# sdoira/U96-SLAM

Hardware: AMD Instinct MI355X
Metric: Mpix-disparities/s (higher is better)
Workload: dtype u8

## Files before the change

### u96-slam_amd/csrc/sbm_api.hip

```cpp
#include <stdio.h>
#include <stdlib.h>
#include <string.h>

#include <algorithm>
#include <mutex>
#include <new>

#include "sbm_handle.h"

using namespace sbm;

enum BmStage { kBmPrefilter, kBmSad, kBmBorder, kBmLr, kBmSpeckle, kBmTotal, kBmStageCount };
enum BmMark { kBmBegin, kBmPrefiltered, kBmMatched, kBmChecked, kBmEnd, kBmMarkCount };
static const char* const kBmNames[] = {"prefilter", "sad", "border", "lrcheck", "speckle", "total"};
StageTable sbm::bm_stages() { return stage_table<kBmStageCount, 0>(kBmNames); }
static_assert(kBmMarkCount == sbm_handle::kMarks, "the ring holds one event per mark");

extern "C" {

void sbm_params_default(sbm_params* p, int num_disparities, int block_size) {
  if (!p) return;
  memset(p, 0, sizeof(*p));
  p->prefilter_type = SBM_PREFILTER_XSOBEL;
  p->prefilter_size = 9;
// ... 346 lines not shown
  if (n <= 0) return SBM_ERR_BATCH;
  const sbm_params& p = h->p;
  BmPlan pl;
  const int st = bm_plan_geom(p, n, width, height, &pl);
  if (st != SBM_OK) return st;
  DeviceScope dscope(h->device);
  HIPCHK(h, dscope.enter());
  bool inplace = false;
  if (pl.in_envelope) HIPCHK(h, mqsad_inplace_ok(h->stream, &inplace));
  bm_plan_launches(p, inplace, &pl);
  const Geom& g = pl.g;
  size_t ho_flags = 0;
  const size_t ho_bytes = sad_fast_handoff_bytes(pl, &ho_flags);
  const int st2 = ensure_scratch(h, n, width, height, g.pitch, g.want_cost, pl.speckle, ho_bytes, ho_flags);
  if (st2 != SBM_OK) return st2;
  h->last = g; h->have_last = true;
  h->bm.ho_links = 0;
  if (pl.any_rows) snprintf(h->last_kernel, sizeof(h->last_kernel), "%s", pl.kernel);

  const uint8_t* dl = (const uint8_t*)d_left;
  const uint8_t* dr = (const uint8_t*)d_right;
  uint8_t *pf_l = h->bm.pf_l.as<uint8_t>(), *pf_r = h->bm.pf_r.as<uint8_t>();
  int16_t* disp_pre = h->bm.disp_pre.as<int16_t>();
  int32_t* cost = h->bm.cost.as<int32_t>();
  int16_t* out = (int16_t*)d_disp;

  h->instr = h->profiling && h->ev_ok && (h->profiling != 3 || (h->ncall & 3u) == 0);
  mark(h, kBmBegin);
  if (pl.any_rows) {
    if (p.prefilter_type == SBM_PREFILTER_XSOBEL) {
      HIPCHK(h, launch_prefilter(dl, dr, pf_l, pf_r, g, h->stream));
    } else {
      HIPCHK(h, h->bm.vsum.grow((size_t)2 * h->bm.n * width * height * sizeof(uint16_t), h->stream));
      HIPCHK(h, launch_prefilter_norm(dl, dr, pf_l, pf_r, h->bm.vsum.as<uint16_t>(), g, p.prefilter_size, h->stream));
    }
  }
  mark(h, kBmPrefiltered);
  if (pl.sad == kSadFast) {
    HIPCHK(h, launch_sad_fast(pf_l, pf_r, disp_pre, cost, pl, ho_bytes ? h->bm.handoff.p : nullptr, ho_bytes ? ++h->bm.ho_epoch : 0u,
                              &h->bm.ho_links, h->stream));
    h->bm.ho_slots = (size_t)h->bm.ho_links;
    if (pl.wide_borders) {
      HIPCHK(h, launch_sad_wide(pf_l, pf_r, disp_pre, cost, g, pl.wide_l[0], pl.wide_l[1], h->stream));
      HIPCHK(h, launch_sad_wide(pf_l, pf_r, disp_pre, cost, g, pl.wide_r[0], pl.wide_r[1], h->stream));
    }
  } else if (pl.sad == kSadWide) {
    HIPCHK(h, launch_sad_wide(pf_l, pf_r, disp_pre, cost, g, 0, g.xend, h->stream));
  } else if (pl.sad == kSadGeneric) {
    HIPCHK(h, launch_sad_generic(pf_l, pf_r, disp_pre, cost, g, 0, g.xend, h->stream));
  }
  mark(h, kBmMatched);
  HIPCHK(h, launch_lrcheck(disp_pre, cost, out, h->bm.lr_keys.as<unsigned long long>(), g, p.disp12_max_diff, h->stream));
  mark(h, kBmChecked);
  if (pl.speckle) HIPCHK(h, launch_speckle(out, h->bm.spk, g, pl.spk, p.speckle_window_size, h->stream));
  mark(h, kBmEnd);
  if (h->instr) h->calls++;
  h->ncall++;
  if (sync || h->profiling == 1) HIPCHK(h, hipStreamSynchronize(h->stream));
  return SBM_OK;
}

int sbm_debug_plan(const sbm_params* p, int n, int width, int height, int inplace_ok, void* out, size_t out_bytes) {
  if (!p || !out) return SBM_ERR_NULL;
  if (out_bytes != sizeof(BmPlan)) return SBM_ERR_SIZE;
  if (n <= 0) return SBM_ERR_BATCH;
  BmPlan pl;
  const int st = bm_plan(*p, n, width, height, inplace_ok != 0, &pl);
  if (st == SBM_OK) memcpy(out, &pl, sizeof(pl));
  return st;
}

int sbm_debug_handoff_bytes(const sbm_params* p, int n, int width, int height, int inplace_ok, uint64_t* out) {
  if (!p || !out) return SBM_ERR_NULL;
  if (n <= 0) return SBM_ERR_BATCH;
  BmPlan pl;
  const int st = bm_plan(*p, n, width, height, inplace_ok != 0, &pl);
  if (st != SBM_OK) return st;
  size_t flags = 0;
  out[0] = sad_fast_handoff_bytes(pl, &flags);
  out[1] = flags;
  return SBM_OK;
}

int sbm_rect_map_device(sbm_handle* h, const sbm_rect_cam* cam, int width, int height, void* d_map, int sync) {
  if (!h || !cam || !d_map) return SBM_ERR_NULL;
  if (width <= 0 || height <= 0 || width > 32767 || height > 32767) return SBM_ERR_SIZE;
  DeviceScope dscope(h->device);
  HIPCHK(h, dscope.enter());
  HIPCHK(h, launch_rect_map(*cam, width, height, (int16_t*)d_map, h->stream));
  if (sync) HIPCHK(h, hipStreamSynchronize(h->stream));
  return SBM_OK;
}

int sbm_rect_remap_device(sbm_handle* h, int n, const void* d_src, const void* d_map, int width, int height, void* d_dst,
                          int sync) {
  if (!h || !d_src || !d_map || !d_dst) return SBM_ERR_NULL;
  if (n <= 0) return SBM_ERR_BATCH;
  if (width <= 0 || height <= 0 || width > 32767 || height > 32767) return SBM_ERR_SIZE;
  if (((size_t)width * height + 1023) / 1024 > 65535) return SBM_ERR_UNSUPPORTED;
  DeviceScope dscope(h->device);
  HIPCHK(h, dscope.enter());
  HIPCHK(h, launch_rect_remap((const uint8_t*)d_src, (const int16_t*)d_map, (uint8_t*)d_dst, n, width, height, h->stream));
  if (sync) HIPCHK(h, hipStreamSynchronize(h->stream));
  return SBM_OK;
}

int sbm_prefilter_device(sbm_handle* h, int n, const void* d_src, int width, int height, int flavour, int cap,
                         void* d_dst, int sync) {
  if (!h || !d_src || !d_dst) return SBM_ERR_NULL;
  if (n <= 0) return SBM_ERR_BATCH;
  if (width <= 0 || height <= 0) return SBM_ERR_SIZE;
  if (flavour != SBM_PREFILTER_FLAVOUR_CV && flavour != SBM_PREFILTER_FLAVOUR_RTL) return SBM_ERR_PREFILTER_TYPE;
  if (flavour == SBM_PREFILTER_FLAVOUR_CV && (cap < 1 || cap > 63)) return SBM_ERR_PREFILTER_CAP;
  if (n > 65534 || height > 65535 * 4) return SBM_ERR_UNSUPPORTED;
  DeviceScope dscope(h->device);
  HIPCHK(h, dscope.enter());
  HIPCHK(h, launch_prefilter_dense((const uint8_t*)d_src, (uint8_t*)d_dst, n, width, height,
                                   flavour == SBM_PREFILTER_FLAVOUR_RTL, cap, h->stream));
  if (sync) HIPCHK(h, hipStreamSynchronize(h->stream));
  return SBM_OK;
}

int sbm_disparity_to_float_device(sbm_handle* h, int n, const void* d_disp, int width, int height, void* d_out, int sync) {
  if (!h || !d_disp || !d_out) return SBM_ERR_NULL;
  if (n <= 0) return SBM_ERR_BATCH;
  if (width <= 0 || height <= 0) return SBM_ERR_SIZE;
  DeviceScope dscope(h->device);
  HIPCHK(h, dscope.enter());
  HIPCHK(h, launch_disp_to_float((const int16_t*)d_disp, (float*)d_out, (size_t)n * width * height, h->stream));
  if (sync) HIPCHK(h, hipStreamSynchronize(h->stream));
  return SBM_OK;
}

int sbm_decimate_device(sbm_handle* h, int n, const void* d_disp, int width, int height, int scale, void* d_out, int sync) {
  if (!h || !d_disp || !d_out) return SBM_ERR_NULL;
  if (n <= 0) return SBM_ERR_BATCH;
  if (width <= 0 || height <= 0 || scale <= 0) return SBM_ERR_SIZE;
  DeviceScope dscope(h->device);
  HIPCHK(h, dscope.enter());
  HIPCHK(h, launch_decimate((const int16_t*)d_disp, (int16_t*)d_out, n, width, height, scale, h->stream));
  if (sync) HIPCHK(h, hipStreamSynchronize(h->stream));
  return SBM_OK;
}

int sbm_reproject_device(sbm_handle* h, int n, const void* d_disp, int width, int height, int scale,
                         const sbm_stereo_model* model, int apply_local, void* d_xyz, int sync) {
  if (!h || !d_disp || !d_xyz || !model) return SBM_ERR_NULL;
  if (n <= 0) return SBM_ERR_BATCH;
  if (width <= 0 || height <= 0 || scale <= 0) return SBM_ERR_SIZE;
  DeviceScope dscope(h->device);
  HIPCHK(h, dscope.enter());
  HIPCHK(h, launch_reproject((const int16_t*)d_disp, (float*)d_xyz, n, width, height, scale, *model, apply_local, h->stream));
  if (sync) HIPCHK(h, hipStreamSynchronize(h->stream));
  return SBM_OK;
}

int sbm_keypoints3d_device(sbm_handle* h, const void* d_disp, int width, int height, const void* d_kpts, int nk,
                           const sbm_stereo_model* model, float min_depth, float max_depth, void* d_xyz, int sync) {
  if (!h || !d_disp || !model || (nk > 0 && (!d_kpts || !d_xyz))) return SBM_ERR_NULL;
  if (width <= 0 || height <= 0 || nk < 0) return SBM_ERR_SIZE;
  DeviceScope dscope(h->device);
  HIPCHK(h, dscope.enter());
  HIPCHK(h, launch_keypoints3d((const int16_t*)d_disp, (const float*)d_kpts, (float*)d_xyz, width, height, nk, *model,
                               min_depth, max_depth, h->stream));
  if (sync) HIPCHK(h, hipStreamSynchronize(h->stream));
  return SBM_OK;
// ... 91 lines not shown
```

### u96-slam_amd/csrc/sbm_common.h

```cpp
#pragma once
#include <hip/hip_runtime.h>
#include <stdint.h>

#include "../../include/sbm.h"
#include "sbm_carve.h"

#include <stdlib.h>

namespace sbm {

inline int env_switch(const char* name, int dflt) {
  const char* e = getenv(name);
  return e ? atoi(e) : dflt;
}

struct Geom {
  int W, H;
  int n;
  int pitch;
  int padl;
  int plane;
  int nd, mindisp, wsz, w2, cap;
  int lofs, rofs, width1, xend;
  int tex, uniq;
  int filtered;
  int row0, row1;
  int col0, col1;
  int want_cost;
  int cost16;
  int pfshift;
  int reading;
};

constexpr int kReadRoiMinusMinD = 1;
constexpr int kReadCostShort = 2;
constexpr int kReadSpeckleX16 = 4;
constexpr int kReadOddRowComputed = 8;
constexpr int kReadLrTieLater = 16;

constexpr int kPfBias = 1;

hipError_t launch_prefilter(const uint8_t* d_left, const uint8_t* d_right, uint8_t* pf_l, uint8_t* pf_r,
                            const Geom& g, hipStream_t s);

hipError_t launch_prefilter_norm(const uint8_t* d_left, const uint8_t* d_right, uint8_t* pf_l, uint8_t* pf_r, uint16_t* vsum,
                                 const Geom& g, int winsize, hipStream_t s);

hipError_t launch_sad_generic(const uint8_t* pf_l, const uint8_t* pf_r, int16_t* disp, int32_t* cost, const Geom& g,
                              int xa, int xb, hipStream_t s);

bool sad_wide_supported(const Geom& g);
hipError_t launch_sad_wide(const uint8_t* pf_l, const uint8_t* pf_r, int16_t* disp, int32_t* cost, const Geom& g, int xa, int xb,
                           hipStream_t s);

enum SadKernel { kSadNone = 0, kSadFast = 1, kSadWide = 2, kSadGeneric = 3 };
struct FastPlan {
  int xc0, xc1;
  int strips, strips3, nseg;
  int segrow[66];
  int split;
  int uniq_plain;
  int NDW, NWAVES, NTERM, PW, exact, dual;
  int bord, bnw, bseg, nbseg;
  int grid, block, lds;
};
struct SpkPlan {
  int lists;
  int G, S, SW, nbands;
  int max_diff;
  int grid[4][2];
};
struct BmPlan {
  Geom g;
  int any_rows;
  int in_envelope;
  int fast;
  int border;
  int speckle;
  int sad;
  int wide_borders;
  int wide_l[2], wide_r[2];
  FastPlan f;
  SpkPlan spk;
  int spk_pad_;
  long long spk_bytes[4];
  char kernel[96];
};
int bm_plan_geom(const sbm_params& p, int n, int W, int H, BmPlan* pl);
void bm_plan_launches(const sbm_params& p, bool inplace_ok, BmPlan* pl);
inline int bm_plan(const sbm_params& p, int n, int W, int H, bool inplace_ok, BmPlan* pl) {
  const int st = bm_plan_geom(p, n, W, H, pl);
  if (st == SBM_OK) bm_plan_launches(p, inplace_ok, pl);
  return st;
}

bool sad_fast_supported(const Geom& g);
hipError_t mqsad_inplace_ok(hipStream_t s, bool* ok);
constexpr int kFastNdMax = 512;
bool sad_fast_borders_in_launch(const Geom& g);
int sad_fast_pfshift(const Geom& g);
void sad_fast_plan(BmPlan* pl);
size_t sad_fast_handoff_bytes(const BmPlan& pl, size_t* flag_bytes);
hipError_t launch_sad_fast(const uint8_t* pf_l, const uint8_t* pf_r, int16_t* disp, int32_t* cost, BmPlan& pl, void* handoff,
                           unsigned epoch, long* links, hipStream_t s);

constexpr int kLrLdsCols = 8192;
inline size_t lr_keys_bytes(int n, int W, int H, bool do_lr) {
  return do_lr && W > kLrLdsCols ? (size_t)n * H * W * sizeof(unsigned long long) : 0;
}
hipError_t launch_lrcheck(const int16_t* disp_pre, const int32_t* cost, int16_t* disp_out, unsigned long long* keys,
                          const Geom& g, int disp12_max_diff, hipStream_t s);

constexpr int kSpkMaxSeg = 4, kSpkRecordPad = 288, kSpkSeamPad = 512;
void speckle_plan(const Geom& g, int max_size, int max_diff, SpkPlan* k);

hipError_t launch_prefilter_dense(const uint8_t* d_src, uint8_t* d_dst, int n, int W, int H, int rtl, int cap,
                                  hipStream_t s);
hipError_t launch_rect_map(const sbm_rect_cam& cam, int W, int H, int16_t* d_map, hipStream_t s);
hipError_t launch_rect_remap(const uint8_t* d_src, const int16_t* d_map, uint8_t* d_dst, int n, int W, int H,
                             hipStream_t s);

hipError_t launch_gftt_eig(const uint8_t* img, uint16_t* eig, unsigned* maxv, int n, int W, int H, hipStream_t s);

hipError_t launch_disp_to_float(const int16_t* disp, float* out, size_t count, hipStream_t s);
hipError_t launch_decimate(const int16_t* disp, int16_t* out, int n, int W, int H, int scale, hipStream_t s);
hipError_t launch_reproject(const int16_t* disp, float* xyz, int n, int W, int H, int scale, const sbm_stereo_model& m,
                            int apply_local, hipStream_t s);
hipError_t launch_keypoints3d(const int16_t* disp, const float* kp, float* xyz, int W, int H, int nk,
                              const sbm_stereo_model& m, float min_depth, float max_depth, hipStream_t s);
hipError_t launch_keypoints3d_lk(const float* kp, const float* rp, const uint8_t* status, const int* count, int n, int cap,
                                 const sbm_stereo_model& m, float min_depth, float max_depth, float* xyz, hipStream_t s);

struct SgbmGeom {
  int W, H, n;
  int minD, D, minX1, maxX1, W1;
  int SW2, P1, P2, ftzero, uniq, d12;
  int fullDP;
  int reading;
};

}
```

### u96-slam_amd/csrc/sbm_sad_fast.hip

```cpp
#include <string.h>

#include "sbm_sad_fast_kernel.h"

namespace sbm {

__global__ void __launch_bounds__(256) mqsad_inplace_selftest_kernel(unsigned* bad) {
  unsigned long long st = (unsigned long long)(blockIdx.x * 256 + threadIdx.x) * 0x9E3779B97F4A7C15ull + 88172645463325252ull;
  auto rnd = [&]() { st ^= st << 13; st ^= st >> 7; st ^= st << 17; return st; };
  unsigned nbad = 0;
  for (int it = 0; it < 64; it++) {
    unsigned long long accA[4], accR[4], win[4];
    const unsigned pat = (unsigned)rnd() & ((it & 1) ? 0x00ffffffu : 0x000000ffu);
#pragma unroll
    for (int q = 0; q < 4; q++) { accA[q] = accR[q] = rnd() & 0x3fff3fff3fff3fffull; win[q] = rnd(); }
#pragma unroll
    for (int r = 0; r < 3; r++)
#pragma unroll
      for (int q = 0; q < 4; q++) {
        accR[q] = __builtin_amdgcn_mqsad_pk_u16_u8(win[(q + r) & 3], pat, accR[q]);
        asm volatile("v_mqsad_pk_u16_u8 %0, %1, %2, %0" : "+v"(accA[q]) : "v"(win[(q + r) & 3]), "v"(pat));
      }
#pragma unroll
    for (int q = 0; q < 4; q++) nbad += accA[q] != accR[q];
  }
// ... 135 lines not shown
  const int ncols = a.xc1 - a.xc0;
  const int nv3 = 64 - (g.wsz / 3 - 1);
  int triples = 0;
  if (pw == 3 && cs3_env) {
    triples = ncols / (3 * nv3);
    if (ncols - triples * 3 * nv3 > 2 * nv) triples++;
  }
  a.strips3 = 3 * triples;
  const int rem = std::max(0, ncols - triples * 3 * nv3);
  const int strips = a.strips3 + (rem + nv - 1) / nv;
  const int rows = g.row1 - g.row0;
  const int round1 = g.nd <= 256 ? 1536 : (g.nd <= 384 ? 1024 : 768);
  constexpr double kSegC = 0.196;
  const int slots_i = g.nd <= 64 ? 4096 : (g.nd <= 128 ? 3072 : round1);
  int nseg = 1;
  {
    const double prime = 0.2 * (g.wsz - 1);
    const double slots = slots_i;
    nseg = (int)(std::sqrt(kSegC * slots * rows / ((double)strips * g.n * prime)) + 0.5);
    nseg = std::max(1, std::min(nseg, std::max(1, rows / g.wsz)));
  }
  constexpr int kSmallRows = 8;
  constexpr long kFill = 5000;
  const int maxseg = std::max(nseg, std::min(64, rows / kSmallRows));
  const long per_seg = (long)strips * g.n;
  if (per_seg * maxseg * (g.nd > 128 ? (g.nd + 127) / 128 : 1) < 1800) {
    nseg = std::max(nseg, (int)std::min<long>(maxseg, 1023 / per_seg));
  } else {
    const int nseg1 = nseg;
    while (per_seg * nseg < kFill && nseg < maxseg) nseg++;
    if (g.nd > 128 && per_seg * nseg > round1 && 2 * per_seg * nseg < 3 * round1) nseg = std::max(nseg1, (int)((long)round1 * 1450 / 1536 / per_seg));
  }
  nseg = std::min(nseg, 64);
  int len[64];
  const int linked = fast_linked_plan(g, rows, per_seg, slots_i, nseg, maxseg, len);
  int ns = 0;
  a.segrow[0] = g.row0;
  if (nseg < 3) {
    const int seg = (rows + nseg - 1) / nseg;
    for (int y = g.row0; y < g.row1; y += seg) a.segrow[++ns] = std::min(y + seg, g.row1);
  } else {
    unsigned char at[64];
    const int stride = fast_segment_order(nseg, per_seg, slots_i, g.nd, at);
    const int first_round = stride - 1;
    if (linked) {
      nseg = linked;
    } else {
      const double step = first_round > 1 ? std::min(kFirstRoundStep, kFirstRoundSpan / (first_round - 1)) : 0.0;
      double wgt[64], sum = 0;
      for (int p = 0; p < nseg; p++) {
        wgt[p] = p < nseg - 3 ? 1.0 : (p == nseg - 3 ? 0.75 : (p == nseg - 2 ? 0.5 : 0.25));
        if (stride < nseg && p < first_round) wgt[p] = std::min(wgt[p], 1.0 - step * (first_round - 1 - p));
        sum += wgt[p];
      }
      const double unit = rows / sum;
      double acc = 0;
      int y0 = 0;
      for (int p = 0; p < nseg; p++) {
        acc += wgt[p] * unit;
        const int y1 = p == nseg - 1 ? rows : std::min(rows, (int)(acc + 0.5));
        len[p] = y1 - y0;
        y0 = y1;
      }
    }
    int np = 0;
    for (int p = 0; p < nseg; p++)
      if (len[p] > 0) len[np++] = len[p];
    fast_segment_order(np, per_seg, slots_i, g.nd, at);
    int seglen[64];
    for (int p = 0; p < np; p++) seglen[at[p]] = len[p];
    for (int k = 0; k < np; k++) a.segrow[k + 1] = a.segrow[k] + seglen[k];
    ns = np;
  }
  nseg = ns;
  a.strips = strips; a.nseg = nseg;
  {
    const long maxs = (long)g.wsz * g.wsz * 2 * g.cap;
    a.uniq_plain = 8 * ((maxs * g.uniq / 100 + 1) << g.pfshift) <= 65535;
  }
  a.split = (long)strips * nseg * g.n < 1024;
  sad_fast_dispatch(*pl, nullptr, nullptr);
}

static unsigned long long fast_handoff_links(const BmPlan& pl, unsigned char* at) {
  const FastPlan& f = pl.f;
  const int mode = fast_handoff_mode();
  const int stride = fast_segment_order(f.nseg, (long)f.strips * pl.g.n, fast_slots(pl.g.nd), pl.g.nd, at);
  if (mode == 0 || f.NWAVES != 1 || !f.exact || f.nseg < 2) return 0;
  unsigned long long links = 0;
  for (int p = mode == 2 ? 1 : stride; p < f.nseg; p++) links |= 1ull << at[p];
  return links;
}

size_t sad_fast_handoff_bytes(const BmPlan& pl, size_t* flag_bytes) {
  unsigned char at[64];
  *flag_bytes = 0;
  if (!pl.fast) return 0;
  const unsigned long long links = fast_handoff_links(pl, at);
  if (!links) return 0;
  size_t fb = 0;
  const size_t bytes = fast_handoff_size(__builtin_popcountll(links), (long)pl.g.n * pl.f.strips, pl.f.NDW, &fb);
  if (bytes > kHandoffMaxBytes) return 0;
  *flag_bytes = fb;
  return bytes;
}

hipError_t launch_sad_fast(const uint8_t* pf_l, const uint8_t* pf_r, int16_t* disp, int32_t* cost, BmPlan& pl, void* handoff,
                           unsigned epoch, long* links, hipStream_t s) {
  const Geom& g = pl.g;
  const FastPlan& f = pl.f;
  FastArgs a;
  a.pf_l = pf_l; a.pf_r = pf_r; a.disp = disp; a.cost = g.want_cost ? reinterpret_cast<uint16_t*>(cost) : nullptr;
  a.W = g.W; a.H = g.H; a.pitch = g.pitch; a.padl = g.padl; a.plane = g.plane;
  a.nd = g.nd; a.mindisp = g.mindisp; a.lofs = g.lofs; a.rofs = g.rofs; a.tex = g.tex << g.pfshift; a.uniq = g.uniq;
  a.filtered = g.filtered; a.capb = (g.cap << g.pfshift) + kPfBias; a.pfshift = g.pfshift;
  a.row0 = g.row0; a.row1 = g.row1;
  static_assert(sizeof(a.segrow) == sizeof(f.segrow), "");
  memcpy(a.segrow, f.segrow, sizeof(a.segrow));
  a.strips = f.strips; a.nseg = f.nseg; a.npairs = g.n; a.strips3 = f.strips3; a.uniq_plain = f.uniq_plain;
  a.xc0 = f.xc0; a.xc1 = f.xc1;
  a.bord = f.bord; a.bnw = f.bnw; a.bseg = f.bseg; a.nbseg = f.nbseg;
  a.ho_link = fast_handoff_links(pl, a.segat);
  if (!handoff) a.ho_link = 0;
  a.ho = static_cast<u32*>(handoff); a.ho_epoch = epoch;
  a.segbase = 0; a.grid = f.grid;
  const long per_seg = (long)f.strips * g.n;
  *links = (long)__builtin_popcountll(a.ho_link) * per_seg;
  if (fast_handoff_mode() != 2 || !a.ho_link) return sad_fast_dispatch(pl, &a, s);
  for (int k = 0; k < f.nseg; k++) {
    a.segbase = k;
    a.grid = (int)per_seg + (k == 0 ? f.bord * f.nbseg : 0);
    if (k == 1) a.bord = 0;
    const hipError_t e = sad_fast_dispatch(pl, &a, s);
    if (e != hipSuccess) return e;
  }
  return hipSuccess;
}

}
```

### u96-slam_amd/csrc/sbm_sad_fast_core.h

```cpp
#pragma once
#include <stdio.h>
#include <stdlib.h>

#include <algorithm>
#include <cmath>
#include <mutex>
#include <type_traits>

#include "sbm_common.h"

namespace sbm {

typedef unsigned int u32;
typedef unsigned long long u64;
typedef unsigned short u16x2 __attribute__((ext_vector_type(2)));
typedef unsigned int u32x4 __attribute__((ext_vector_type(4)));
typedef unsigned int u32x2 __attribute__((ext_vector_type(2)));

struct FastArgs {
  const uint8_t* pf_l;
  const uint8_t* pf_r;
  int16_t* disp;
  uint16_t* cost;
  int W, H, pitch, padl, plane;
  int nd, mindisp, lofs, rofs, tex, uniq, filtered, capb;
  int row0, row1;
  int segrow[66];
  int strips, nseg, npairs;
  unsigned char segat[64];
  int grid;
  int segbase;
  unsigned long long ho_link;
  u32* ho;
  u32 ho_epoch;
  int strips3;
  int uniq_plain;
  int xc0, xc1;
  int pfshift;
  int bord;
  int bnw;
  int bseg, nbseg;
};

__device__ __forceinline__ u32 pk_sub_sat(u32 a, u32 b) {
  u16x2 r = __builtin_elementwise_sub_sat(__builtin_bit_cast(u16x2, a), __builtin_bit_cast(u16x2, b));
  return __builtin_bit_cast(u32, r);
}
__device__ __forceinline__ u32 pk_add_sat(u32 a, u32 b) {
  u16x2 r = __builtin_elementwise_add_sat(__builtin_bit_cast(u16x2, a), __builtin_bit_cast(u16x2, b));
  return __builtin_bit_cast(u32, r);
}
__device__ __forceinline__ u32 pk_min(u32 a, u32 b) {
  u16x2 r = __builtin_elementwise_min(__builtin_bit_cast(u16x2, a), __builtin_bit_cast(u16x2, b));
  return __builtin_bit_cast(u32, r);
}
__device__ __forceinline__ u32 umin3(u32 a, u32 b, u32 c) {
  u32 r;
  asm("v_min3_u32 %0, %1, %2, %3" : "=v"(r) : "v"(a), "v"(b), "v"(c));
  return r;
}

constexpr int kHandoffAux = 16;
template <int NDW, int NWAVES, bool EXACT_ND>
struct FastHandoff {
  static constexpr bool ON = NWAVES == 1 && EXACT_ND;
  static constexpr int SLOT_B = (NDW / 4) * 512 + 256;
};

extern __shared__ __attribute__((aligned(16))) uint4 fast_lds[];

#include "sbm_sad_border_wave.h"

constexpr int kFastPrioExchange = 2;

template <int NDW, int NTERM, int PW, int CS>
struct FastLds {
  static constexpr int NQ = NDW / 4;
  static constexpr int NCH = (NQ + 15) / 16;
  static constexpr int NSLOT = ((CS * 63 + 4 + 16 * (4 * (NCH - 1) + 3) + 1) + 63) / 64 * 64;
  static constexpr int KS = CS == 3 ? 1 : PW;
  static constexpr int XS = 64 + KS * (NTERM - 1);
  static_assert(CS == 1 || (CS == 3 && PW == 3), "column stride 3 goes with 3-column sums");
};

template <int NTERM, int PW>
struct HPlan {
  static constexpr int S1 = NTERM >= 23 ? 5 : (NTERM == 17 ? 4 : (NTERM >= 7 ? 3 : 1));
  static constexpr int NTT = S1 > 1 ? NTERM / S1 : 0;
  static constexpr int NVV = NTERM - NTT * S1;
  static constexpr bool PUB1 = NTT >= 2;
  static constexpr int NLEV = 1 + PUB1;
};

template <int NDW, int NWAVES, int NTERM, int PW, int CS>
struct DmaLds {
  using L = FastLds<NDW, NTERM, PW, CS>;
  using P = HPlan<NTERM, PW>;
  static constexpr int XCH = 2;
  static_assert(L::NQ >= XCH, "a wavefront holds at least two disparity quads");
  static constexpr int STAGE_B = L::NSLOT * 4;
  static constexpr int XLEV_B = ((XCH / 2) * L::XS + (L::XS * 4 + 15) / 16) * 16;
  static constexpr int PAT_OFS = STAGE_B > XLEV_B ? STAGE_B : XLEV_B;
  static constexpr int AREA_B = PAT_OFS + 256;
  static constexpr int WAVE_B = 2 * AREA_B + (P::NLEV - 1) * XLEV_B;
};


template <int WSZ>
struct FastTag {
  static constexpr int BITS = WSZ <= 15 ? 2 : 1;
  static constexpr int NGRP = 1 << BITS;
  static __device__ __forceinline__ u32 tag_unit(const int pfshift) { return pfshift == BITS ? 0x00010001u : 0u; }
};
template <int NR, int WSZ>
__device__ __forceinline__ u32 fast_first_min(const u32 (&S)[NR], const int pfshift) {
  u32 best = 0xffffffffu;
  constexpr int TSMAX = FastTag<WSZ>::BITS;
  if (NR >= 16 && TSMAX == 2 && pfshift == 2) {
    constexpr int NG = NR / 4;
    u32 b[4] = {0xffffffffu, 0xffffffffu, 0xffffffffu, 0xffffffffu};
#pragma unroll
    for (int j = 0; j < NG; j++) {
      const u32 g01 = pk_min(S[j], S[j + NG]);
      const u32 g23 = pk_min(S[j + 2 * NG], S[j + 3 * NG]);
      const u32 gm = pk_min(g01, g23);
      const u32 klo = (gm << 16) | (u32)(2 * j);
      const u32 khi = (gm & 0xffff0000u) | (u32)(2 * j + 1);
      b[j & 3] = umin3(b[j & 3], klo, khi);
    }
    const u32 bt = min(min(b[0], b[1]), min(b[2], b[3]));
    best = (bt & 0xfffc0000u) | (((bt >> 16) & 3u) * (u32)(2 * NG) + (bt & 0xffffu));
  } else if (NR >= 16 && TSMAX == 1 && pfshift == 1) {
    constexpr int NG = NR / 2;
    u32 b[4] = {0xffffffffu, 0xffffffffu, 0xffffffffu, 0xffffffffu};
#pragma unroll
    for (int j = 0; j < NG; j++) {
      const u32 gm = pk_min(S[j], S[j + NG]);
      const u32 klo = (gm << 16) | (u32)(2 * j);
      const u32 khi = (gm & 0xffff0000u) | (u32)(2 * j + 1);
      b[j & 3] = umin3(b[j & 3], klo, khi);
    }
    const u32 bt = min(min(b[0], b[1]), min(b[2], b[3]));
    best = (bt & 0xfffe0000u) | (((bt >> 16) & 1u) * (u32)(2 * NG) + (bt & 0xffffu));
  } else {
#pragma unroll
    for (int g0 = 0; g0 < NR; g0 += 32) {
      u32 b[4] = {0xffffffffu, 0xffffffffu, 0xffffffffu, 0xffffffffu};
#pragma unroll
      for (int j = g0; j < g0 + 32 && j < NR; j++) {
        const u32 klo = (S[j] << 16) | (u32)(2 * (j - g0));
        const u32 khi = (S[j] & 0xffff0000u) | (u32)(2 * (j - g0) + 1);
        b[j & 3] = umin3(b[j & 3], klo, khi);
      }
      const u32 bg = min(min(b[0], b[1]), min(b[2], b[3])) + (u32)(2 * g0);
      best = min(best, bg);
    }
  }
  return best;
}

__device__ __forceinline__ u32 fast_uniq_threshold(const int minsad, const int uniq, const int pfshift) {
  const int ms = minsad >> pfshift;
  const int thresh = ms + (ms * uniq / 100);
  return (u32)min((thresh + 1) << pfshift, 65536 - (1 << pfshift));
}

template <int NR, int WSZ>
__device__ __forceinline__ u32 fast_deficits(const u32 (&S)[NR], const u32 T, const int uniq_plain, const int pfshift) {
  constexpr int NGRP = FastTag<WSZ>::NGRP, NG = NR / NGRP;
  const u32 tg = FastTag<WSZ>::tag_unit(pfshift);
  const u32 T2 = T | (T << 16);
  constexpr int NACC = NR >= 32 ? NR / 8 : 4;
  u32 ac[NACC];
#pragma unroll
  for (int k = 0; k < NACC; k++) ac[k] = 0u;
  if (uniq_plain) {
#pragma unroll
    for (int g = 0; g < NGRP; g++) {
      const u32 Tg = T2 + (u32)g * tg;
#pragma unroll
      for (int j = g * NG; j < (g + 1) * NG; j++) ac[j % NACC] += pk_sub_sat(Tg, S[j]);
    }
  } else {
    u32 T2s = T2;
    asm("" : "+v"(T2s));
#pragma unroll
    for (int g = 0; g < NGRP; g++) {
      const u32 Tg = T2s + (u32)g * tg;
#pragma unroll
// ... 55 lines not shown
```

### u96-slam_amd/csrc/sbm_sad_fast_kernel.h

```cpp
#pragma once
#include "sbm_sad_fast_core.h"
#include "sbm_sad_fast_strip.h"

namespace sbm {

template <int NDW, int NWAVES, int NTERM, int PW, bool EXACT_ND, bool DUAL>
__global__ void __launch_bounds__(64 * NWAVES) __attribute__((amdgpu_waves_per_eu(NDW > 64 ? 3 : (NWAVES > 2 ? 5 : 4))))
sad_fast_kernel(FastArgs a) {
  const int bpp = a.strips;
  int strip, segi, pair;
  {
    if constexpr (NDW * NWAVES <= 256) {
    if ((int)blockIdx.x < a.bord * a.nbseg) {
      using BL = BorderLds<(PW * NTERM) / 2, NDW * NWAVES>;
      const int bseg = blockIdx.x / a.bord, b = blockIdx.x - bseg * a.bord;
      const int wv = NWAVES > 1 ? __builtin_amdgcn_readfirstlane(threadIdx.x >> 6) : 0;
      const int wi = b * NWAVES + wv;
      if (wi < a.bnw) sad_border_wave<(PW * NTERM) / 2, NDW * NWAVES>(a, reinterpret_cast<unsigned char*>(fast_lds) + wv * BL::BYTES, bseg, wi);
      return;
    }
    }
    const int sid = blockIdx.x - a.bord * a.nbseg;
    const int per_seg = a.strips * a.npairs;
    const int pos = sid / per_seg;
    segi = a.segat[a.segbase + pos];
    const int b = sid - pos * per_seg;
    const int full = (a.npairs / 8) * 8 * bpp;
    int p, inner;
    if (b < full) {
      const int xcd = b & 7, k = b >> 3;
      p = (k / bpp) * 8 + xcd;
      inner = k % bpp;
    } else {
      const int r = b - full;
      p = (a.npairs / 8) * 8 + r / bpp;
      inner = r % bpp;
    }
    pair = p;
    strip = inner;
  }
  const int wvk = NWAVES > 1 ? __builtin_amdgcn_readfirstlane(threadIdx.x >> 6) : 0;
  unsigned char* const ldsb = reinterpret_cast<unsigned char*>(fast_lds);
  auto strip_at = [&](auto cs_tag, const int cb) {
    constexpr int CSV = decltype(cs_tag)::value;
    using D = DmaLds<NDW, NWAVES, NTERM, PW, CSV>;
    unsigned char* const wb = ldsb + wvk * D::WAVE_B;
    unsigned char* const xl = wb + 2 * D::AREA_B;
    sad_fast_strip_dma<NDW, NWAVES, NTERM, PW, EXACT_ND, CSV>(a, wb, wb + D::AREA_B, xl,
                                                            reinterpret_cast<u32*>(ldsb + NWAVES * D::WAVE_B), cb, segi, pair, strip);
  };
  if constexpr (DUAL) {
    constexpr int NV3 = 64 - (NTERM - 1), NV1 = 64 - PW * (NTERM - 1);
    if (strip < a.strips3) {
      const int t = strip / 3;
      strip_at(std::integral_constant<int, 3>{}, t * (3 * NV3) + (strip - 3 * t));
    } else {
      strip_at(std::integral_constant<int, 1>{}, (a.strips3 / 3) * (3 * NV3) + (strip - a.strips3) * NV1);
    }
  } else {
    constexpr int NV1 = 64 - PW * (NTERM - 1);
    strip_at(std::integral_constant<int, 1>{}, strip * NV1);
  }
}

constexpr double kBorderModelRate = 3.6e12, kBorderRowUs = 2.0, kBorderColUs = 0.25, kBorderChainShare = 0.205;

template <int NDW, int NWAVES, int NTERM, int PW>
static hipError_t launch_t(BmPlan& pl, const FastArgs* a, hipStream_t s) {
  constexpr bool DUAL = PW == 3;
  constexpr bool HAS_EXACT = !(NDW == 64 && NWAVES == 4);
  if (!a) {
    FastPlan& f = pl.f;
    const Geom& g = pl.g;
    constexpr int WB1 = DmaLds<NDW, NWAVES, NTERM, PW, 1>::WAVE_B, WB3 = DmaLds<NDW, NWAVES, NTERM, PW, DUAL ? 3 : 1>::WAVE_B;
    size_t lds = (size_t)NWAVES * (WB1 > WB3 ? WB1 : WB3) + (NWAVES > 1 ? (size_t)2 * NWAVES * 64 * (4 + 8) : 0);
    f.bord = f.bnw = 0;
    f.bseg = g.row1 - g.row0;
    f.nbseg = 0;
    if constexpr (NDW * NWAVES <= 256) if (pl.border) {
      using BL = BorderLds<(PW * NTERM) / 2, NDW * NWAVES>;
      f.bnw = 2 * ((g.n + BL::JW - 1) / BL::JW);
      f.bord = (f.bnw + NWAVES - 1) / NWAVES;
      lds = std::max(lds, (size_t)NWAVES * BL::BYTES);
      const int rows = g.row1 - g.row0, wsz = PW * NTERM;
      const double t_kernel_us = (double)g.n * g.W * rows * g.nd / kBorderModelRate * 1e6;
      const double t_row_us = kBorderRowUs + kBorderColUs * (wsz / 2);
      int bseg = (int)(kBorderChainShare * t_kernel_us / t_row_us - 0.25 * (wsz - 1));
      bseg = std::max(4, std::min(bseg, rows));
      f.nbseg = (rows + bseg - 1) / bseg;
      f.bseg = (rows + f.nbseg - 1) / f.nbseg;
      f.nbseg = (rows + f.bseg - 1) / f.bseg;
    }
    f.grid = f.bord * f.nbseg + f.strips * g.n * f.nseg;
    f.block = 64 * NWAVES;
    f.lds = (int)lds;
    f.NDW = NDW; f.NWAVES = NWAVES; f.NTERM = NTERM; f.PW = PW; f.dual = DUAL;
    f.exact = HAS_EXACT && g.nd == NDW * NWAVES;
    snprintf(pl.kernel, sizeof(pl.kernel), "sad_fast_kernel<%d,%d,%d,%d,%s,%s> pfshift=%d",
             NDW, NWAVES, NTERM, PW, f.exact ? "true" : "false", DUAL ? "true" : "false", g.pfshift);
    return hipSuccess;
  }
  const dim3 grid((unsigned)a->grid);
  const size_t lds = (size_t)pl.f.lds;
  if constexpr (HAS_EXACT) {
    if (pl.f.exact) {
      hipLaunchKernelGGL((sad_fast_kernel<NDW, NWAVES, NTERM, PW, true, DUAL>), grid, dim3(64 * NWAVES), lds, s, *a);
      return hipGetLastError();
    }
  }
    hipLaunchKernelGGL((sad_fast_kernel<NDW, NWAVES, NTERM, PW, false, DUAL>), grid, dim3(64 * NWAVES), lds, s, *a);
  return hipGetLastError();
}

template <int NTERM, int PW>
static hipError_t launch_nd(BmPlan& pl, const FastArgs* a, hipStream_t s) {
  const int nd = pl.g.nd;
  const bool split = pl.f.split;
  if (nd > 384) return launch_t<128, 4, NTERM, PW>(pl, a, s);
  if (nd > 256) return launch_t<128, 3, NTERM, PW>(pl, a, s);
  if (nd <= 32) return launch_t<32, 1, NTERM, PW>(pl, a, s);
  if (nd <= 64) return split ? launch_t<32, 2, NTERM, PW>(pl, a, s) : launch_t<64, 1, NTERM, PW>(pl, a, s);
  if (!split && nd <= 128) return launch_t<128, 1, NTERM, PW>(pl, a, s);
  if (!split && nd != 192) return launch_t<128, 2, NTERM, PW>(pl, a, s);
  if (nd <= 128) return launch_t<64, 2, NTERM, PW>(pl, a, s);
  if (nd <= 192) return launch_t<64, 3, NTERM, PW>(pl, a, s);
  return launch_t<64, 4, NTERM, PW>(pl, a, s);
}

hipError_t launch_sad_fast_pw1(BmPlan& pl, const FastArgs* a, hipStream_t s);
hipError_t launch_sad_fast_pw2(BmPlan& pl, const FastArgs* a, hipStream_t s);
hipError_t launch_sad_fast_pw3(BmPlan& pl, const FastArgs* a, hipStream_t s);

}
```

Before: 4.442 million.

## Fold the final narrow SAD strip into a half-wave two-row kernel path

Adds a specialised path for the last single-pass strip when only a few output columns remain. Each wave half covers 64 of the 128 disparities for 32 columns, and the halves are combined with permlane32 swaps. The aim is to avoid spending a full 64-column strip's worth of SAD work on a small leftover, at the cost of a new intricate code path with its own LDS layout and handoff handling. It is on by default (SBM_FAST_FOLD=1) but only fires for NDW=128, one wave, exact nd, window 15, dual mode.

After: 4.501 million (median of 6 runs). +1.3%, better.

```diff
diff --git a/u96-slam_amd/csrc/sbm_api.hip b/u96-slam_amd/csrc/sbm_api.hip
--- a/u96-slam_amd/csrc/sbm_api.hip
+++ b/u96-slam_amd/csrc/sbm_api.hip
@@ -452,6 +452,16 @@
   return SBM_OK;
 }
 
+int sbm_debug_fold(const sbm_params* p, int n, int width, int height, int inplace_ok, int* out) {
+  if (!p || !out) return SBM_ERR_NULL;
+  if (n <= 0) return SBM_ERR_BATCH;
+  BmPlan pl;
+  const int st = bm_plan(*p, n, width, height, inplace_ok != 0, &pl);
+  if (st != SBM_OK) return st;
+  out[0] = sad_fast_fold_cols(pl);
+  return SBM_OK;
+}
+
 int sbm_rect_map_device(sbm_handle* h, const sbm_rect_cam* cam, int width, int height, void* d_map, int sync) {
   if (!h || !cam || !d_map) return SBM_ERR_NULL;
   if (width <= 0 || height <= 0 || width > 32767 || height > 32767) return SBM_ERR_SIZE;
diff --git a/u96-slam_amd/csrc/sbm_common.h b/u96-slam_amd/csrc/sbm_common.h
--- a/u96-slam_amd/csrc/sbm_common.h
+++ b/u96-slam_amd/csrc/sbm_common.h
@@ -100,6 +100,7 @@
 bool sad_fast_borders_in_launch(const Geom& g);
 int sad_fast_pfshift(const Geom& g);
 void sad_fast_plan(BmPlan* pl);
+int sad_fast_fold_cols(const BmPlan& pl);
 size_t sad_fast_handoff_bytes(const BmPlan& pl, size_t* flag_bytes);
 hipError_t launch_sad_fast(const uint8_t* pf_l, const uint8_t* pf_r, int16_t* disp, int32_t* cost, BmPlan& pl, void* handoff,
                            unsigned epoch, long* links, hipStream_t s);
diff --git a/u96-slam_amd/csrc/sbm_sad_fast.hip b/u96-slam_amd/csrc/sbm_sad_fast.hip
--- a/u96-slam_amd/csrc/sbm_sad_fast.hip
+++ b/u96-slam_amd/csrc/sbm_sad_fast.hip
@@ -241,6 +241,16 @@
   sad_fast_dispatch(*pl, nullptr, nullptr);
 }
 
+int sad_fast_fold_cols(const BmPlan& pl) {
+  const FastPlan& f = pl.f;
+  if (!pl.fast || env_switch("SBM_FAST_FOLD", 1) == 0) return 0;
+  if (f.NDW != FoldLds::NDW || f.NWAVES != 1 || !f.exact || f.NTERM * f.PW != FoldLds::NTERM * FoldLds::PW || !f.dual) return 0;
+  if (f.strips <= f.strips3) return 0;
+  const int nv3 = 64 - (f.NTERM - 1), nv1 = 64 - f.PW * (f.NTERM - 1);
+  const int cols = (f.xc1 - f.xc0) - ((f.strips3 / 3) * 3 * nv3 + (f.strips - 1 - f.strips3) * nv1);
+  return cols >= 1 && cols <= FoldLds::NV ? cols : 0;
+}
+
 static unsigned long long fast_handoff_links(const BmPlan& pl, unsigned char* at) {
   const FastPlan& f = pl.f;
   const int mode = fast_handoff_mode();
@@ -278,6 +288,7 @@
   memcpy(a.segrow, f.segrow, sizeof(a.segrow));
   a.strips = f.strips; a.nseg = f.nseg; a.npairs = g.n; a.strips3 = f.strips3; a.uniq_plain = f.uniq_plain;
   a.xc0 = f.xc0; a.xc1 = f.xc1;
+  a.fold = sad_fast_fold_cols(pl) > 0;
   a.bord = f.bord; a.bnw = f.bnw; a.bseg = f.bseg; a.nbseg = f.nbseg;
   a.ho_link = fast_handoff_links(pl, a.segat);
   if (!handoff) a.ho_link = 0;
diff --git a/u96-slam_amd/csrc/sbm_sad_fast_core.h b/u96-slam_amd/csrc/sbm_sad_fast_core.h
--- a/u96-slam_amd/csrc/sbm_sad_fast_core.h
+++ b/u96-slam_amd/csrc/sbm_sad_fast_core.h
@@ -34,6 +34,7 @@
   u32* ho;
   u32 ho_epoch;
   int strips3;
+  int fold;
   int uniq_plain;
   int xc0, xc1;
   int pfshift;
@@ -105,6 +106,23 @@
   static constexpr int WAVE_B = 2 * AREA_B + (P::NLEV - 1) * XLEV_B;
 };
 
+struct FoldLds {
+  using Plain = DmaLds<128, 1, 5, 3, 1>;
+  static constexpr int NDW = 128, NTERM = 3, PW = 5, KS = 5;
+  static constexpr int NQ = NDW / 2 / 4;
+  static constexpr int NV = 32 - KS * (NTERM - 1);
+  static constexpr int NSLOT = ((31 + NDW / 2 + 4 * (NQ - 1) + 8 + 1) + 63) / 64 * 64;
+  static constexpr int XS = 64 + KS * (NTERM - 1);
+  static constexpr int XCH = 2;
+  static constexpr int STAGE_B = NSLOT * 4;
+  static constexpr int XLEV_B = ((XCH / 2) * XS + (XS * 4 + 15) / 16) * 16;
+  static constexpr int PAT_OFS = STAGE_B > XLEV_B ? STAGE_B : XLEV_B;
+  static constexpr int AREA_B = PAT_OFS + 256;
+  static constexpr int WAVE_B = 2 * AREA_B;
+  static_assert(NSLOT == 192 && XS == 74, "the folded strip stages 192 dword slots and exchanges 74 entries");
+  static_assert(NSLOT <= Plain::L::NSLOT && WAVE_B <= Plain::WAVE_B, "the folded strip fits the plain strip's LDS");
+};
+
 
 template <int WSZ>
 struct FastTag {
diff --git a/u96-slam_amd/csrc/sbm_sad_fast_fold.h b/u96-slam_amd/csrc/sbm_sad_fast_fold.h
--- /dev/null
+++ b/u96-slam_amd/csrc/sbm_sad_fast_fold.h
@@ -0,0 +1,234 @@
+#pragma once
+#include "sbm_sad_fast_core.h"
+
+namespace sbm {
+
+__device__ __forceinline__ void sad_fast_strip_fold(const FastArgs& a, unsigned char* __restrict__ const b0c, unsigned char* __restrict__ const b1c,
+                                                    const int cbase, const int segi, const int pair, const int strip) {
+  using D = FoldLds;
+  typedef __attribute__((address_space(3))) void* lds_vptr;
+  constexpr int NQ = D::NQ;
+  constexpr int NR = 2 * NQ;
+  constexpr int NIT = D::NSLOT / 64;
+  constexpr int WSZ = D::PW * D::NTERM, W2 = WSZ / 2;
+  constexpr int KS = D::KS, XCH = D::XCH, XS = D::XS;
+  constexpr int SLOT_B = FastHandoff<D::NDW, 1, true>::SLOT_B;
+
+  const int lane = threadIdx.x & 63;
+  const unsigned lane_u = (unsigned)lane;
+  const int col = lane & 31;
+  const u32 half = lane_u >> 5;
+  const int c = cbase + col;
+  const int xc = c + W2;
+  const bool produces = col < D::NV && xc >= a.xc0 && xc < a.xc1;
+  const int ys = a.segrow[segi];
+  const int ye = a.segrow[segi + 1];
+  const uint8_t* pl = a.pf_l + (size_t)pair * a.plane + a.padl + a.lofs + cbase;
+  const uint8_t* pr = a.pf_r + (size_t)pair * a.plane + a.padl + a.rofs + cbase;
+  const __amdgpu_buffer_rsrc_t rs_l = __builtin_amdgcn_make_buffer_rsrc(const_cast<uint8_t*>(pl), 0, 0x7fffffff, 0x00020000);
+  const __amdgpu_buffer_rsrc_t rs_r = __builtin_amdgcn_make_buffer_rsrc(const_cast<uint8_t*>(pr), 0, 0x7fffffff, 0x00020000);
+  uint4* const b0 = reinterpret_cast<uint4*>(b0c);
+  uint4* const b1 = reinterpret_cast<uint4*>(b1c);
+  uint4* const xq0 = b0;
+  u32* const xt0 = reinterpret_cast<u32*>(xq0 + (XCH / 2) * XS);
+  const u32 capw = (u32)a.capb * 0x01010101u;
+
+  u64 VB[NQ];
+  {
+    const u32 unit = ((unsigned)col / (unsigned)KS) % (unsigned)D::NTERM == 0u ? FastTag<WSZ>::tag_unit(a.pfshift) : 0u;
+#pragma unroll
+    for (int q = 0; q < NQ; q++) {
+      const u32 tq = (u32)((2 * q) / (NR / FastTag<WSZ>::NGRP)) * unit;
+      VB[q] = __builtin_bit_cast(u64, make_uint2(tq, tq));
+    }
+  }
+  u32 Vt = 0;
+
+  auto pat_of = [](uint4* const buf) { return reinterpret_cast<u32*>(reinterpret_cast<unsigned char*>(buf) + D::PAT_OFS); };
+  auto stage = [&](const int y, uint4* const buf) {
+    const int rowoff = __builtin_amdgcn_readfirstlane(y * a.pitch);
+#pragma unroll
+    for (int it = 0; it < NIT; it++)
+      __builtin_amdgcn_raw_ptr_buffer_load_lds(rs_r, (lds_vptr)(reinterpret_cast<u32*>(buf) + 64 * it), 4, (int)lane_u, rowoff + 64 * it, 0, 0);
+    __builtin_amdgcn_raw_ptr_buffer_load_lds(rs_l, (lds_vptr)pat_of(buf), 4, (int)lane_u, rowoff, 0, 0);
+  };
+  auto landed = [] {
+    __builtin_amdgcn_s_waitcnt(0);
+    __builtin_amdgcn_fence(__ATOMIC_ACQUIRE, "wavefront");
+    __builtin_amdgcn_wave_barrier();
+  };
+  auto reads_done = [] {
+    __builtin_amdgcn_s_waitcnt(0xc07f);
+    __builtin_amdgcn_wave_barrier();
+  };
+  auto published = [] {
+    __builtin_amdgcn_fence(__ATOMIC_RELEASE, "wavefront");
+    __builtin_amdgcn_wave_barrier();
+  };
+  auto apply = [&](uint4* const buf, const bool leave) {
+    const u32 pat4 = pat_of(buf)[col];
+    const u32 pat1 = pat_of(buf)[col + 4] & 0xffu;
+    const u32 tv = __builtin_amdgcn_sad_u8(pat1 | (capw & ~0xffu), capw, __builtin_amdgcn_sad_u8(pat4, capw, 0u));
+    const u32* const win4 = reinterpret_cast<const u32*>(buf) + col + 64 * (int)half;
+    u32 lo[NQ], mi[NQ], mj[NQ], hi[NQ];
+#pragma unroll
+    for (int q = 0; q < NQ; q++) { lo[q] = win4[4 * q]; mi[q] = win4[4 * q + 4]; }
+#pragma unroll
+    for (int q = 0; q < NQ; q++) { mj[q] = win4[4 * q + 4]; hi[q] = win4[4 * q + 8]; }
+#pragma unroll
+    for (int q = 0; q < NQ; q++) {
+      const u64 w0 = ((u64)mi[q] << 32) | lo[q], w1 = ((u64)hi[q] << 32) | mj[q];
+      if (!leave) {
+        asm("v_mqsad_pk_u16_u8 %0, %1, %2, %0" : "+v"(VB[q]) : "v"(w0), "v"(pat4));
+        asm("v_mqsad_pk_u16_u8 %0, %1, %2, %0" : "+v"(VB[q]) : "v"(w1), "v"(pat1));
+      } else {
+        const u64 t0 = __builtin_amdgcn_mqsad_pk_u16_u8(w0, pat4, 0ull);
+        const uint2 tt = __builtin_bit_cast(uint2, __builtin_amdgcn_mqsad_pk_u16_u8(w1, pat1, t0));
+        uint2 vb = __builtin_bit_cast(uint2, VB[q]);
+        vb.x -= tt.x;
+        vb.y -= tt.y;
+        asm("" : "+v"(vb.x), "+v"(vb.y));
+        VB[q] = __builtin_bit_cast(u64, vb);
+      }
+    }
+    Vt = leave ? Vt - tv : Vt + tv;
+  };
+
+  const size_t ho_set = (size_t)a.npairs * a.strips;
+  const size_t ho_slots = (size_t)__builtin_popcountll(a.ho_link) * ho_set;
+  auto ho_slot = [&](const int k) { return (size_t)__builtin_popcountll(a.ho_link & ((1ull << k) - 1)) * ho_set + (size_t)pair * a.strips + strip; };
+  auto ho_rsrc = [&](const size_t slot) {
+    unsigned char* const p = reinterpret_cast<unsigned char*>(a.ho) + ((2 * ho_slots * sizeof(u32) + 255) & ~(size_t)255) + slot * SLOT_B;
+    return __builtin_amdgcn_make_buffer_rsrc(p, 0, NQ * 512 + 256, 0x00020000);
+  };
+  bool take = false;
+  if ((a.ho_link >> segi) & 1) {
+    const size_t from = ho_slot(segi);
+    take = __builtin_amdgcn_readfirstlane(__hip_atomic_load(a.ho + from, __ATOMIC_RELAXED, __HIP_MEMORY_SCOPE_AGENT)) == a.ho_epoch;
+    if (take) {
+      __builtin_amdgcn_fence(__ATOMIC_ACQUIRE, "agent");
+      const __amdgpu_buffer_rsrc_t rs_h = ho_rsrc(from);
+#pragma unroll
+      for (int q = 0; q < NQ; q++) VB[q] = __builtin_bit_cast(u64, __builtin_amdgcn_raw_buffer_load_b64(rs_h, (int)(8 * lane_u), 512 * q, kHandoffAux));
+      Vt = __builtin_amdgcn_raw_buffer_load_b32(rs_h, (int)(4 * lane_u), 512 * NQ, kHandoffAux);
+      if (lane == 0) a.ho[ho_slots + from] = a.ho_epoch;
+      stage(ys + W2, b0);
+    }
+  }
+  if (!take) {
+    stage(ys - W2, b0);
+    for (int i = 0; i < 2 * W2; i += 2) {
+      landed();
+      stage(ys - W2 + i + 1, b1);
+      apply(b0, false);
+      landed();
+      stage(ys - W2 + i + 2, b0);
+      apply(b1, false);
+    }
+  }
+  const __amdgpu_buffer_rsrc_t rs_d = __builtin_amdgcn_make_buffer_rsrc(a.disp + (size_t)pair * a.W * a.H, 0, 0x7fffffff, 0x00020000);
+  const __amdgpu_buffer_rsrc_t rs_c = __builtin_amdgcn_make_buffer_rsrc(a.cost + (size_t)pair * a.W * a.H, 0, 0x7fffffff, 0x00020000);
+  const int ocol_u = __builtin_amdgcn_readfirstlane(2 * (a.lofs + cbase + W2));
+  const bool stores = produces && half == 0u;
+  u32 res_prev = 0xffff0000u;
+  auto flush = [&](const int yrow) {
+    if (stores) {
+      const int orow_prev = __builtin_amdgcn_readfirstlane(2 * yrow * a.W) + ocol_u;
+      const int ocol = 2 * col;
+      if (a.cost) __builtin_amdgcn_raw_buffer_store_b16((short)(res_prev >> 16), rs_c, ocol, orow_prev, 0);
+      __builtin_amdgcn_raw_buffer_store_b16((short)res_prev, rs_d, ocol, orow_prev, 0);
+    }
+  };
+  for (int y = ys; y < ye; y++) {
+    landed();
+    if (y > ys) {
+      flush(y - 1);
+      apply(b1, true);
+    }
+    reads_done();
+    stage(y - W2, b1);
+    apply(b0, false);
+
+    __builtin_amdgcn_s_setprio(kFastPrioExchange);
+    u32 S[NR];
+    unsigned long long tex_ok = 0;
+    u32 lx = lane_u;
+    asm volatile("" : "+v"(lx));
+#pragma unroll
+    for (int q0 = 0; q0 < NQ; q0 += XCH) {
+      const bool tex_now = q0 == 0;
+      const uint2 v0 = __builtin_bit_cast(uint2, VB[q0]), v1 = __builtin_bit_cast(uint2, VB[q0 + 1]);
+      xq0[lane] = make_uint4(v0.x, v0.y, v1.x, v1.y);
+      if (tex_now) xt0[lane] = Vt;
+      published();
+      const uint4 r1 = xq0[lx + KS], r2 = xq0[lx + 2 * KS];
+      S[2 * q0 + 0] = v0.x + r1.x + r2.x;
+      S[2 * q0 + 1] = v0.y + r1.y + r2.y;
+      S[2 * q0 + 2] = v1.x + r1.z + r2.z;
+      S[2 * q0 + 3] = v1.y + r1.w + r2.w;
+      if (tex_now) {
+        const u32 tA = Vt + xt0[lx + KS] + xt0[lx + 2 * KS];
+        tex_ok = __ballot((int)tA >= a.tex);
+      }
+      __builtin_amdgcn_wave_barrier();
+    }
+    reads_done();
+    stage(min(y + 1 + W2, a.H - 1), b0);
+    __builtin_amdgcn_s_setprio(0);
+
+    u32 best = fast_first_min<NR, WSZ>(S, a.pfshift) + 64u * half;
+    {
+      const auto r = __builtin_amdgcn_permlane32_swap(best, best, false, false);
+      best = min(r[0], r[1]);
+    }
+    const int minsad = (int)(best >> 16), mind = (int)(best & 0xffffu);
+
+    u32 acc = 0, T = 0;
+    if (a.uniq > 0) {
+      T = fast_uniq_threshold(minsad, a.uniq, a.pfshift);
+      acc = fast_deficits<NR, WSZ>(S, T, a.uniq_plain, a.pfshift);
+      const auto r = __builtin_amdgcn_permlane32_swap(acc, acc, false, false);
+      acc = pk_add_sat(r[0], r[1]);
+    }
+
+    const int in_ = mind > 0 ? mind - 1 : 1;
+    const int ip_ = mind < a.nd - 1 ? mind + 1 : a.nd - 2;
+    const int d0 = 64 * (int)half;
+    const int ln = min(max(in_ - d0, 0), 63), lp = min(max(ip_ - d0, 0), 63);
+    int nn, pp;
+    {
+      u32 X[NQ];
+      const u32 lnp = (u32)ln | ((u32)lp << 16);
+      fast_neighbours_quads<NQ>(S, lnp, X);
+      const u32 X0 = fast_neighbours_tree<NQ>(X, lnp) & ~(((1u << a.pfshift) - 1u) * 0x00010001u);
+      const auto r = __builtin_amdgcn_permlane32_swap(X0, X0, false, false);
+      nn = (int)((in_ >= 64 ? r[1] : r[0]) & 0xffffu);
+      pp = (int)((ip_ >= 64 ? r[1] : r[0]) >> 16);
+    }
+
+    bool ok = __builtin_amdgcn_inverse_ballot_w64(tex_ok);
+    if (a.uniq > 0) ok = ok && fast_unique(acc & 0xffffu, acc >> 16, T, minsad, mind, nn, pp, a.nd);
+    if (stores) {
+      int out = a.filtered, cst = -1;
+      if (ok) {
+        out = fast_subpixel(nn, pp, minsad, mind, a.nd, a.mindisp);
+        if (a.cost) cst = minsad >> a.pfshift;
+      }
+      res_prev = ((u32)out & 0xffffu) | ((u32)cst << 16);
+    }
+  }
+  flush(ye - 1);
+  if (segi + 1 < a.nseg && ((a.ho_link >> (segi + 1)) & 1)) {
+    landed();
+    apply(b1, true);
+    const size_t ho_mine = ho_slot(segi + 1);
+    const __amdgpu_buffer_rsrc_t rs_h = ho_rsrc(ho_mine);
+#pragma unroll
+    for (int q = 0; q < NQ; q++) __builtin_amdgcn_raw_buffer_store_b64(__builtin_bit_cast(u32x2, VB[q]), rs_h, (int)(8 * lane_u), 512 * q, kHandoffAux);
+    __builtin_amdgcn_raw_buffer_store_b32(Vt, rs_h, (int)(4 * lane_u), 512 * NQ, kHandoffAux);
+    asm volatile("s_waitcnt vmcnt(0)" ::: "memory");
+    if (lane == 0) __hip_atomic_store(a.ho + ho_mine, a.ho_epoch, __ATOMIC_RELAXED, __HIP_MEMORY_SCOPE_AGENT);
+  }
+}
+
+}
diff --git a/u96-slam_amd/csrc/sbm_sad_fast_kernel.h b/u96-slam_amd/csrc/sbm_sad_fast_kernel.h
--- a/u96-slam_amd/csrc/sbm_sad_fast_kernel.h
+++ b/u96-slam_amd/csrc/sbm_sad_fast_kernel.h
@@ -1,6 +1,7 @@
 #pragma once
 #include "sbm_sad_fast_core.h"
 #include "sbm_sad_fast_strip.h"
+#include "sbm_sad_fast_fold.h"
 
 namespace sbm {
 
@@ -55,7 +56,14 @@
       const int t = strip / 3;
       strip_at(std::integral_constant<int, 3>{}, t * (3 * NV3) + (strip - 3 * t));
     } else {
-      strip_at(std::integral_constant<int, 1>{}, (a.strips3 / 3) * (3 * NV3) + (strip - a.strips3) * NV1);
+      const int cb = (a.strips3 / 3) * (3 * NV3) + (strip - a.strips3) * NV1;
+      if constexpr (NDW == FoldLds::NDW && NWAVES == 1 && EXACT_ND && NTERM * PW == FoldLds::NTERM * FoldLds::PW) {
+        if (a.fold && strip == a.strips - 1) {
+          sad_fast_strip_fold(a, ldsb, ldsb + FoldLds::AREA_B, cb, segi, pair, strip);
+          return;
+        }
+      }
+      strip_at(std::integral_constant<int, 1>{}, cb);
     }
   } else {
     constexpr int NV1 = 64 - PW * (NTERM - 1);
```
